# IuvenisSapiens/Qwen3-TTS-Rust

Measured on AMD Instinct MI355X. Metric: audio-seconds generated per second (aggregate over GPUs) = concurrent real-time streams; RTF and first-chunk latency from the single-utterance leg, higher is better.
Workload: dtype i8

## Files before the change

qwen3-tts-rust_amd/csrc/codec.hip:

```cpp
#include "codec.h"
#include "../../include/q3tts.h"
#include "gguf.h"
#include <cmath>
#include <cstdlib>
#include <map>

namespace q3 {

typedef float f32x16 __attribute__((ext_vector_type(16)));

enum { EPI_NONE = 0, EPI_GELU = 1, EPI_RES_SCALE = 2, EPI_RES = 3, EPI_SNAKE = 4 };

struct GemmArgs {
    const float* A; int lda;
    int cin, dil;
    const float* W;
    const float* wscale;
    const float* bias;
    float* out; int ldo;
    int M, N, K;
    int epi; const float* res; int ldr; const float* scale;
    const float *snake_ea, *snake_ib;
    float* ws;
    int a_segT, a_skip; int o_segT; long long o_skip; int r_segT; long long r_skip;
// ... 124 lines not shown
            const int e = tid + i * 256, r = e % BN, qd = e / BN;
            if (e < BN * 4) { Bs[4 * qd + 0][r] = rb[i].x; Bs[4 * qd + 1][r] = rb[i].y; Bs[4 * qd + 2][r] = rb[i].z; Bs[4 * qd + 3][r] = rb[i].w; }
        }
    };
    fetch(kbeg);
    for (int k0 = kbeg; k0 < kend; k0 += BK) {
        stash();
        __syncthreads();
        if (k0 + BK < kend) fetch(k0 + BK);
#pragma unroll
        for (int kk = 0; kk < BK; kk += 2) {
            const float a = As[kk + (lane >> 5)][wm * 32 + (lane & 31)];
            const float b = Bs[kk + (lane >> 5)][wn * 32 + (lane & 31)];
            acc = __builtin_amdgcn_mfma_f32_32x32x2f32(a, b, acc, 0, 0, 0);
        }
        __syncthreads();
    }
    const int col = n0 + wn * 32 + (lane & 31);
    if (col < g.N) {
#pragma unroll
        for (int r = 0; r < 16; r++) {
            const int row = m0 + wm * 32 + (r & 3) + 8 * (r >> 2) + 4 * (lane >> 5);
            if (row < g.M) {
                if (ksplit > 1) g.ws[((size_t)blockIdx.z * g.M + row) * g.N + col] = acc[r];
                else gemm_store(g, row, col, gemm_epilogue(g, acc[r], row, col));
            }
        }
    }
}
typedef _Float16 h8v __attribute__((ext_vector_type(8)));
typedef _Float16 h4v __attribute__((ext_vector_type(4)));
template <int MR, int EPL, bool SPLIT>
__global__ void __launch_bounds__(256) k_conv_gemm_h(GemmArgs g, const _Float16* __restrict__ Wh, const _Float16* __restrict__ Wl) {
    constexpr int BM = 64 * MR, BN = 64, BK = 32, LD = 40;
    constexpr int NA = BM * 8 / 256;
    constexpr int CLD = BN + 4;
    struct Stage { _Float16 Ah[BM][LD], Al[BM][LD], Bh[BN][LD], Bl[BN][LD]; };
    union Shared { Stage s; float Ct[EPL ? BM : 1][CLD]; };
    __shared__ __attribute__((aligned(16))) Shared sh;
    auto& Ah = sh.s.Ah; auto& Al = sh.s.Al; auto& Bh = sh.s.Bh; auto& Bl = sh.s.Bl;
    const int tid = threadIdx.x, lane = tid & 63, wave = tid >> 6;
    const int wm = wave >> 1, wn = wave & 1;
    const int m0 = blockIdx.y * BM, n0 = blockIdx.x * BN;
    const int ksplit = gridDim.z, kper = g.K / ksplit, kbeg = blockIdx.z * kper, kend = kbeg + kper;
    f32x16 acc[MR];
#pragma unroll
    for (int t = 0; t < MR; t++)
#pragma unroll
        for (int i = 0; i < 16; i++) acc[t][i] = 0.0f;
    float4 ra[NA];
    uint4 rh, rl;
    int arow[NA];
#pragma unroll
    for (int i = 0; i < NA; i++) { int mm = m0 + (tid + i * 256) / 8; mm = mm < g.M ? mm : g.M - 1; arow[i] = mm + seg_of(mm, g.a_segT) * g.a_skip; }
    const int wrow = (n0 + tid / 4 < g.N) ? n0 + tid / 4 : g.N - 1, wk = 8 * (tid & 3);
    const int scol = n0 + wn * 32 + (lane & 31);
    const float wsc = g.wscale[scol < g.N ? scol : g.N - 1];
    auto fetch = [&](int k0) {
        const int j = k0 / g.cin, ci0 = k0 % g.cin;
#pragma unroll
        for (int i = 0; i < NA; i++) {
            const int kq = (tid + i * 256) % 8;
            const size_t row = (size_t)(arow[i] + j * g.dil);
            if constexpr (SPLIT) ra[i] = load_a4_split_raw(g, row, ci0 + 4 * kq);
            else ra[i] = *reinterpret_cast<const float4*>(g.A + row * g.lda + ci0 + 4 * kq);
        }
        rh = *reinterpret_cast<const uint4*>(Wh + (size_t)wrow * g.K + k0 + wk);
        rl = *reinterpret_cast<const uint4*>(Wl + (size_t)wrow * g.K + k0 + wk);
    };
    auto stash = [&]() {
#pragma unroll
        for (int i = 0; i < NA; i++) {
            const int e = tid + i * 256, r = e / 8, kq = e % 8;
            if constexpr (SPLIT) {
                *reinterpret_cast<float2*>(&Ah[r][4 * kq]) = make_float2(ra[i].x, ra[i].y);
                *reinterpret_cast<float2*>(&Al[r][4 * kq]) = make_float2(ra[i].z, ra[i].w);
            } else {
                const float x[4] = {ra[i].x, ra[i].y, ra[i].z, ra[i].w};
                h4v hi, lo;
#pragma unroll
                for (int c = 0; c < 4; c++) { hi[c] = (_Float16)x[c]; lo[c] = (_Float16)(x[c] - (float)hi[c]); }
                *reinterpret_cast<h4v*>(&Ah[r][4 * kq]) = hi;
                *reinterpret_cast<h4v*>(&Al[r][4 * kq]) = lo;
            }
        }
        *reinterpret_cast<uint4*>(&Bh[tid / 4][wk]) = rh;
        *reinterpret_cast<uint4*>(&Bl[tid / 4][wk]) = rl;
    };
    auto multiply = [&]() {
#pragma unroll
        for (int kk = 0; kk < BK; kk += 16) {
            const int ko = kk + 8 * (lane >> 5);
            const h8v bh = *reinterpret_cast<const h8v*>(&Bh[wn * 32 + (lane & 31)][ko]);
            const h8v bl = *reinterpret_cast<const h8v*>(&Bl[wn * 32 + (lane & 31)][ko]);
#pragma unroll
            for (int t = 0; t < MR; t++) {
                const int ar = (wm * MR + t) * 32 + (lane & 31);
                const h8v ah = *reinterpret_cast<const h8v*>(&Ah[ar][ko]);
                const h8v al = *reinterpret_cast<const h8v*>(&Al[ar][ko]);
                acc[t] = __builtin_amdgcn_mfma_f32_32x32x16_f16(al, bh, acc[t], 0, 0, 0);
                acc[t] = __builtin_amdgcn_mfma_f32_32x32x16_f16(ah, bl, acc[t], 0, 0, 0);
                acc[t] = __builtin_amdgcn_mfma_f32_32x32x16_f16(ah, bh, acc[t], 0, 0, 0);
            }
        }
    };
    auto lds_barrier = [] { asm volatile("s_waitcnt lgkmcnt(0)\n\ts_barrier" ::: "memory"); };
    fetch(kbeg);
    int k0 = kbeg;
    for (; k0 + BK < kend; k0 += BK) {
        stash();
        lds_barrier();
        fetch(k0 + BK);
        multiply();
        lds_barrier();
    }
    stash();
    lds_barrier();
    multiply();
#pragma unroll
    for (int t = 0; t < MR; t++)
#pragma unroll
        for (int r = 0; r < 16; r++) acc[t][r] *= wsc;
    __syncthreads();
    if constexpr (EPL != 0) {
        auto& Ct = sh.Ct;
#pragma unroll
        for (int t = 0; t < MR; t++)
#pragma unroll
            for (int r = 0; r < 16; r++) Ct[(wm * MR + t) * 32 + (r & 3) + 8 * (r >> 2) + 4 * (lane >> 5)][wn * 32 + (lane & 31)] = acc[t][r];
        __syncthreads();
        for (int e = tid; e < BM * (BN / 4); e += 256) {
            const int rl = e / (BN / 4), cl = (e % (BN / 4)) * 4, row = m0 + rl, col = n0 + cl;
            if (row >= g.M || col >= g.N) continue;
            const float4 t4 = *reinterpret_cast<const float4*>(&Ct[rl][cl]);
            if (ksplit > 1) *reinterpret_cast<float4*>(g.ws + ((size_t)blockIdx.z * g.M + row) * g.N + col) = t4;
            else gemm_epilogue_store4(g, t4, row, col);
        }
    } else {
        const int col = n0 + wn * 32 + (lane & 31);
        if (col < g.N) {
#pragma unroll
            for (int t = 0; t < MR; t++)
#pragma unroll
                for (int r = 0; r < 16; r++) {
                    const int row = m0 + (wm * MR + t) * 32 + (r & 3) + 8 * (r >> 2) + 4 * (lane >> 5);
                    if (row < g.M) {
                        if (ksplit > 1) g.ws[((size_t)blockIdx.z * g.M + row) * g.N + col] = acc[t][r];
                        else gemm_store(g, row, col, gemm_epilogue(g, acc[t][r], row, col));
                    }
                }
        }
    }
}
template <int MR, int NT, int BK, int EPL, int PF, bool SPLIT>
__global__ void __launch_bounds__(256) k_conv_gemm_h3(GemmArgs g, const _Float16* __restrict__ Wh, const _Float16* __restrict__ Wl) {
    constexpr int BM = 128 * MR, BN = 32 * NT, LD = BK + 8;
    constexpr int KQ = BK / 4, KC = BK / 8;
    constexpr int NA = BM * KQ / 256;
    constexpr int NB = (BN * KC + 255) / 256;
    constexpr int CLD = BN + 4;
    struct Stage { _Float16 Ah[BM][LD], Al[BM][LD], Bh[BN][LD], Bl[BN][LD]; };
    union Shared { Stage s; float Ct[EPL ? BM : 1][CLD]; };
    __shared__ __attribute__((aligned(16))) Shared sh;
    auto& Ah = sh.s.Ah; auto& Al = sh.s.Al; auto& Bh = sh.s.Bh; auto& Bl = sh.s.Bl;
    const int tid = threadIdx.x, lane = tid & 63, wave = tid >> 6;
    int tile_m = blockIdx.y, tile_n = blockIdx.x;
    if (g.xcd_swizzle) {
        const int nwg = gridDim.x * gridDim.y, orig = blockIdx.y * gridDim.x + blockIdx.x;
        const int xcd = orig & 7, q8 = nwg >> 3, r8 = nwg & 7;
        const int wgid = (xcd < r8 ? xcd * (q8 + 1) : r8 * (q8 + 1) + (xcd - r8) * q8) + (orig >> 3);
        tile_n = wgid % gridDim.x; tile_m = wgid / gridDim.x;
    }
    const int m0 = tile_m * BM, n0 = tile_n * BN;
    const int ksplit = gridDim.z, kper = g.K / ksplit, kbeg = blockIdx.z * kper, kend = kbeg + kper;
    f32x16 acc[MR][NT];
#pragma unroll
    for (int t = 0; t < MR; t++)
#pragma unroll
        for (int u = 0; u < NT; u++)
#pragma unroll
            for (int i = 0; i < 16; i++) acc[t][u][i] = 0.0f;
    int arow[NA];
#pragma unroll
    for (int i = 0; i < NA; i++) { int mm = m0 + (tid + i * 256) / KQ; mm = mm < g.M ? mm : g.M - 1; arow[i] = mm + seg_of(mm, g.a_segT) * g.a_skip; }
    struct Regs { float4 ra[NA]; uint4 rh[NB], rl[NB]; };
    auto fetch = [&](Regs& s, int k0) {
        const int j = k0 / g.cin, ci0 = k0 % g.cin;
#pragma unroll
        for (int i = 0; i < NA; i++) {
            const int kq = (tid + i * 256) % KQ;
            const size_t row = (size_t)(arow[i] + j * g.dil);
            if constexpr (SPLIT) s.ra[i] = load_a4_split_raw(g, row, ci0 + 4 * kq);
            else s.ra[i] = *reinterpret_cast<const float4*>(g.A + row * g.lda + ci0 + 4 * kq);
        }
#pragma unroll
        for (int i = 0; i < NB; i++) {
            int e = tid + i * 256;
            e = e < BN * KC ? e : e - 256;
            const int r = e / KC, wk = 8 * (e % KC);
            s.rh[i] = *reinterpret_cast<const uint4*>(Wh + (size_t)(n0 + r) * g.K + k0 + wk);
            s.rl[i] = *reinterpret_cast<const uint4*>(Wl + (size_t)(n0 + r) * g.K + k0 + wk);
        }
    };
    auto stash = [&](const Regs& s) {
#pragma unroll
        for (int i = 0; i < NA; i++) {
            const int e = tid + i * 256, r = e / KQ, kq = e % KQ;
            if constexpr (SPLIT) {
                *reinterpret_cast<float2*>(&Ah[r][4 * kq]) = make_float2(s.ra[i].x, s.ra[i].y);
                *reinterpret_cast<float2*>(&Al[r][4 * kq]) = make_float2(s.ra[i].z, s.ra[i].w);
            } else {
                const float x[4] = {s.ra[i].x, s.ra[i].y, s.ra[i].z, s.ra[i].w};
                h4v hi, lo;
#pragma unroll
                for (int c = 0; c < 4; c++) { hi[c] = (_Float16)x[c]; lo[c] = (_Float16)(x[c] - (float)hi[c]); }
                *reinterpret_cast<h4v*>(&Ah[r][4 * kq]) = hi;
                *reinterpret_cast<h4v*>(&Al[r][4 * kq]) = lo;
            }
        }
#pragma unroll
        for (int i = 0; i < NB; i++) {
            const int e = tid + i * 256, r = e / KC, wk = 8 * (e % KC);
            if (e < BN * KC) { *reinterpret_cast<uint4*>(&Bh[r][wk]) = s.rh[i]; *reinterpret_cast<uint4*>(&Bl[r][wk]) = s.rl[i]; }
        }
    };
    auto multiply = [&]() {
#pragma unroll
        for (int kk = 0; kk < BK; kk += 16) {
            const int ko = kk + 8 * (lane >> 5);
            if constexpr (MR == 1) {
                const int ar = wave * 32 + (lane & 31);
                const h8v ah = *reinterpret_cast<const h8v*>(&Ah[ar][ko]);
                const h8v al = *reinterpret_cast<const h8v*>(&Al[ar][ko]);
#pragma unroll
                for (int u = 0; u < NT; u++) {
                    const h8v bh = *reinterpret_cast<const h8v*>(&Bh[u * 32 + (lane & 31)][ko]);
                    const h8v bl = *reinterpret_cast<const h8v*>(&Bl[u * 32 + (lane & 31)][ko]);
                    acc[0][u] = __builtin_amdgcn_mfma_f32_32x32x16_f16(al, bh, acc[0][u], 0, 0, 0);
                    acc[0][u] = __builtin_amdgcn_mfma_f32_32x32x16_f16(ah, bl, acc[0][u], 0, 0, 0);
                    acc[0][u] = __builtin_amdgcn_mfma_f32_32x32x16_f16(ah, bh, acc[0][u], 0, 0, 0);
                }
            } else {
                h8v bh[NT], bl[NT];
#pragma unroll
                for (int u = 0; u < NT; u++) {
                    bh[u] = *reinterpret_cast<const h8v*>(&Bh[u * 32 + (lane & 31)][ko]);
                    bl[u] = *reinterpret_cast<const h8v*>(&Bl[u * 32 + (lane & 31)][ko]);
                }
#pragma unroll
                for (int t = 0; t < MR; t++) {
                    const int ar = (wave * MR + t) * 32 + (lane & 31);
                    const h8v ah = *reinterpret_cast<const h8v*>(&Ah[ar][ko]);
                    const h8v al = *reinterpret_cast<const h8v*>(&Al[ar][ko]);
#pragma unroll
                    for (int u = 0; u < NT; u++) {
                        acc[t][u] = __builtin_amdgcn_mfma_f32_32x32x16_f16(al, bh[u], acc[t][u], 0, 0, 0);
                        acc[t][u] = __builtin_amdgcn_mfma_f32_32x32x16_f16(ah, bl[u], acc[t][u], 0, 0, 0);
                        acc[t][u] = __builtin_amdgcn_mfma_f32_32x32x16_f16(ah, bh[u], acc[t][u], 0, 0, 0);
                    }
                    __builtin_amdgcn_sched_barrier(0);
                }
            }
        }
    };
    auto lds_barrier = [] { asm volatile("s_waitcnt lgkmcnt(0)\n\ts_barrier" ::: "memory"); };
    float wsc[NT];
#pragma unroll
    for (int u = 0; u < NT; u++) wsc[u] = g.wscale[n0 + u * 32 + (lane & 31)];
    Regs st[PF];
#pragma unroll
    for (int j = 0; j < PF; j++)
        if (kbeg + j * BK < kend) fetch(st[j], kbeg + j * BK);
    int k0 = kbeg;
    for (; k0 + 2 * PF * BK <= kend; k0 += PF * BK) {
#pragma unroll
        for (int j = 0; j < PF; j++) {
            stash(st[j]);
            lds_barrier();
            fetch(st[j], k0 + (j + PF) * BK);
            multiply();
            lds_barrier();
        }
    }
    for (; k0 < kend; k0 += PF * BK) {
#pragma unroll
        for (int j = 0; j < PF; j++) {
            if (k0 + j * BK < kend) {
                stash(st[j]);
                lds_barrier();
                if (k0 + (j + PF) * BK < kend) fetch(st[j], k0 + (j + PF) * BK);
                multiply();
                lds_barrier();
            }
        }
    }
#pragma unroll
    for (int u = 0; u < NT; u++)
#pragma unroll
        for (int t = 0; t < MR; t++)
#pragma unroll
            for (int r = 0; r < 16; r++) acc[t][u][r] *= wsc[u];
    __syncthreads();
    auto epilogue_rows = [&](const f32x16 (&a)[NT], int row0) {
#pragma unroll
        for (int r = 0; r < 16; r++) {
            const int row = row0 + (r & 3) + 8 * (r >> 2) + 4 * (lane >> 5);
            if (row < g.M) {
#pragma unroll
                for (int u = 0; u < NT; u++) {
                    const int col = n0 + u * 32 + (lane & 31);
                    if (col < g.N) {
                        if (ksplit > 1) g.ws[((size_t)blockIdx.z * g.M + row) * g.N + col] = a[u][r];
                        else gemm_store(g, row, col, gemm_epilogue(g, a[u][r], row, col));
                    }
                }
            }
        }
    };
    if constexpr (EPL != 0 && MR == 1) {
        auto& Ct = sh.Ct;
#pragma unroll
        for (int u = 0; u < NT; u++)
#pragma unroll
            for (int r = 0; r < 16; r++) Ct[wave * 32 + (r & 3) + 8 * (r >> 2) + 4 * (lane >> 5)][u * 32 + (lane & 31)] = acc[0][u][r];
        __syncthreads();
        constexpr int C4 = BN / 4;
        for (int e = tid; e < BM * C4; e += 256) {
            const int rl = e / C4, col = n0 + (e % C4) * 4, row = m0 + rl;
            if (row >= g.M) continue;
            const float4 t4 = *reinterpret_cast<const float4*>(&Ct[rl][(e % C4) * 4]);
            if (ksplit > 1) *reinterpret_cast<float4*>(g.ws + ((size_t)blockIdx.z * g.M + row) * g.N + col) = t4;
            else gemm_epilogue_store4(g, t4, row, col);
        }
    } else {
        epilogue_rows(acc[0], m0 + wave * MR * 32);
        if constexpr (MR > 1) epilogue_rows(acc[1], m0 + (wave * MR + 1) * 32);
    }
    static_assert(MR <= 2, "one epilogue call per row tile");
}
__global__ void __launch_bounds__(256) k_splitk_reduce4(GemmArgs g, int ksplit) {
    const size_t i = ((size_t)blockIdx.x * 256 + threadIdx.x) * 4, mn = (size_t)g.M * g.N;
    if (i >= mn) return;
    const int row = (int)(i / g.N), col = (int)(i % g.N);
    float4 v = *reinterpret_cast<const float4*>(g.ws + i);
    for (int s = 1; s < ksplit; s++) {
        const float4 w = *reinterpret_cast<const float4*>(g.ws + (size_t)s * mn + i);
        v.x += w.x; v.y += w.y; v.z += w.z; v.w += w.w;
    }
    gemm_epilogue_store4(g, v, row, col);
}
__global__ void __launch_bounds__(256) k_splitk_reduce(GemmArgs g, int ksplit) {
    const size_t i = (size_t)blockIdx.x * 256 + threadIdx.x;
    if (i >= (size_t)g.M * g.N) return;
    const int row = (int)(i / g.N), col = (int)(i % g.N);
    float v = g.ws[i];
    for (int s = 1; s < ksplit; s++) v += g.ws[(size_t)s * g.M * g.N + i];
    gemm_store(g, row, col, gemm_epilogue(g, v, row, col));
}

template <int MT>
__global__ void __launch_bounds__(512) k_skinny_gemm(GemmArgs g) {
    constexpr int KT = 512;
    __shared__ __attribute__((aligned(16))) float As[MT][KT];
    const int tid = threadIdx.x, lane = tid & 63, wave = tid >> 6;
    const int n = blockIdx.x * 8 + wave;
    const int nn = n < g.N ? n : g.N - 1;
    float acc[MT];
#pragma unroll
    for (int m = 0; m < MT; m++) acc[m] = 0.0f;
    for (int k0 = 0; k0 < g.K; k0 += KT) {
        const int kt = (g.K - k0) < KT ? (g.K - k0) : KT;
        float4 w4[2];
#pragma unroll
        for (int i = 0; i < 2; i++) {
            const int kk = 4 * (lane + 64 * i);
            w4[i] = (kk < kt) ? *reinterpret_cast<const float4*>(g.W + (size_t)nn * g.K + k0 + kk) : make_float4(0.f, 0.f, 0.f, 0.f);
        }
        __syncthreads();
        for (int e = tid; e < MT * (KT / 4); e += 512) {
            const int m = e / (KT / 4), kk = 4 * (e % (KT / 4));
            float4 v = make_float4(0.f, 0.f, 0.f, 0.f);
            if (m < g.M && kk < kt) {
                const int kg = k0 + kk, j = kg / g.cin, ci = kg % g.cin;
                v = load_a4(g, (size_t)(m + seg_of(m, g.a_segT) * g.a_skip + j * g.dil), ci);
            }
            *reinterpret_cast<float4*>(&As[m][kk]) = v;
        }
        __syncthreads();
#pragma unroll
        for (int i = 0; i < 2; i++) {
            const int kk = 4 * (lane + 64 * i);
#pragma unroll
            for (int m = 0; m < MT; m++) {
                const float4 a = *reinterpret_cast<const float4*>(&As[m][kk]);
                acc[m] += w4[i].x * a.x + w4[i].y * a.y + w4[i].z * a.z + w4[i].w * a.w;
            }
        }
    }
    float mine = 0.0f;
#pragma unroll
    for (int m = 0; m < MT; m++) {
        float v = acc[m];
        for (int o = 32; o >= 1; o >>= 1) v += __shfl_xor(v, o);
        if (lane == m) mine = v;
    }
    if (lane < MT && lane < g.M && n < g.N) gemm_store(g, lane, n, gemm_epilogue(g, mine, lane, n));
}
static const bool g_codec_f32 = [] { const char* e = std::getenv("Q3_CODEC_F32"); return e && e[0] == '1'; }();
struct GemmPlan { int form, ks, red; };
static GemmPlan plan_gemm(const GemmArgs& g, size_t ws_floats, bool has_split_w) {
    if (g.M <= 16) return GemmPlan{g.M <= 4 ? Q3TTS_GEMM_SKINNY4 : g.M <= 8 ? Q3TTS_GEMM_SKINNY8 : Q3TTS_GEMM_SKINNY16, 1, -1};
    const bool small = g.M <= 32;
    const int tiles = small ? ((g.N + 127) / 128) * ((g.M + 31) / 32) : ((g.N + 63) / 64) * ((g.M + 63) / 64);
    int ksplit = 1;
    while (tiles * ksplit < 256 && ksplit < 16 && (g.K / (ksplit * 2)) % 16 == 0 && g.K / (ksplit * 2) >= 128 &&
           (size_t)(ksplit * 2) * g.M * g.N <= ws_floats) ksplit *= 2;
    const bool ws_a16 = (reinterpret_cast<uintptr_t>(g.ws) & 15) == 0;
    static const int h3_min_wgs = [] { const char* e = std::getenv("Q3_CODEC_H3_MIN_WGS"); return e ? atoi(e) : 128; }();
    static const int h3_max_n = [] { const char* e = std::getenv("Q3_CODEC_H3_MAXN"); return e ? atoi(e) : 1 << 30; }();
    static const int epl_on = [] { const char* e = std::getenv("Q3_CODEC_H3_EPL"); return e ? atoi(e) : 1; }();
    static const int h3_wgs = [] { const char* e = std::getenv("Q3_CODEC_H3_WGS"); return e ? atoi(e) : 0; }();
    static const int h3_min_tiles = [] { const char* e = std::getenv("Q3_CODEC_H3_MIN_TILES"); return e ? atoi(e) : 96; }();
    if (!small && has_split_w && !g_codec_f32 && g.cin % 32 == 0 && h3_min_wgs > 0 && g.N % 96 == 0 && g.N <= h3_max_n) {
        const int tiles3 = (g.N / 96) * ((g.M + 127) / 128);
        const bool vec_ok = epl_on && epilogue4_ok(g) && ws_a16;
        int ks = 1;
        if (vec_ok && h3_wgs > 0 && tiles3 >= h3_min_tiles && tiles3 < h3_wgs) {
            static const int cand[] = {2, 3, 4, 6, 7, 8, 12, 14, 16};
            for (int c : cand) {
                if (g.K % c != 0 || (g.K / c) % 32 != 0 || g.K / c < 256 || (size_t)c * g.M * g.N > ws_floats) continue;
                ks = c;
                if (tiles3 * c >= h3_wgs) break;
            }
        }
        if (tiles3 * ks >= h3_min_wgs) return GemmPlan{vec_ok ? Q3TTS_GEMM_H3_EPL : Q3TTS_GEMM_H3, ks, ks > 1 ? 1 : -1};
    }
    if (!small && has_split_w && !g_codec_f32 && g.cin % 32 == 0) {
        static const int big_m = [] { const char* e = std::getenv("Q3_CODEC_BM128"); return e ? atoi(e) : 1024; }();
        const bool tall = g.M >= big_m && g.N >= 512 && ((g.N + 63) / 64) * ((g.M + 127) / 128) >= 160;
        const int t2 = tall ? ((g.N + 63) / 64) * ((g.M + 127) / 128) : tiles;
        static const int wg_target = [] { const char* e = std::getenv("Q3_CODEC_WGS"); return e ? atoi(e) : 256; }();
        int ks = 1;
        while (t2 * ks < wg_target && ks < 16 && (g.K / (ks * 2)) % 32 == 0 && g.K / (ks * 2) >= 128 && (size_t)(ks * 2) * g.M * g.N <= ws_floats) ks *= 2;
        static const int epl4 = [] { const char* e = std::getenv("Q3_CODEC_EPL4"); return e ? atoi(e) : 1; }();
        const bool vec_ok = epl4 && epilogue4_ok(g) && ws_a16;
        const int form = tall ? (vec_ok ? Q3TTS_GEMM_H2_EPL : Q3TTS_GEMM_H2) : (vec_ok ? Q3TTS_GEMM_H1_EPL : Q3TTS_GEMM_H1);
        return GemmPlan{form, ks, ks > 1 ? (vec_ok ? 1 : 0) : -1};
    }
    return GemmPlan{small ? Q3TTS_GEMM_F32_1 : Q3TTS_GEMM_F32_2, ksplit, ksplit > 1 ? 0 : -1};
}
static const char* gemm_plan_error(const GemmArgs& g, const GemmPlan& p, size_t ws_floats, bool has_split_w) {
    const int f = p.form;
    if (f < Q3TTS_GEMM_SKINNY4 || f > Q3TTS_GEMM_H3_EPL) return "unknown GEMM form";
    if (g.M < 1 || g.N < 1 || g.cin < 4 || g.K % g.cin != 0 || g.dil < 1) return "bad GEMM shape";
    if (g.cin % 4 != 0 || g.lda % 4 != 0 || g.lda < g.cin) return "A rows need cin % 4 == 0 and lda % 4 == 0, lda >= cin";
    if (p.ks < 1 || g.K % p.ks != 0) return "ksplit must divide K";
    const bool skinny = f <= Q3TTS_GEMM_SKINNY16, f32 = f == Q3TTS_GEMM_F32_1 || f == Q3TTS_GEMM_F32_2, h3 = f >= Q3TTS_GEMM_H3;
    const bool epl = f == Q3TTS_GEMM_H1_EPL || f == Q3TTS_GEMM_H2_EPL || f == Q3TTS_GEMM_H3_EPL;
    const bool ws_a16 = (reinterpret_cast<uintptr_t>(g.ws) & 15) == 0;
    if (skinny) {
        if (g.M > (f == Q3TTS_GEMM_SKINNY4 ? 4 : f == Q3TTS_GEMM_SKINNY8 ? 8 : 16)) return "skinny form: M exceeds its row count";
        if (p.ks != 1) return "skinny form: no split-K";
        return nullptr;
    }
    if (f32 && (g.cin % 16 != 0 || (g.K / p.ks) % 16 != 0)) return "f32 form: cin and K / ksplit must be multiples of 16";
    if (!f32) {
        if (!has_split_w || !g.wscale) return "split-f16 form without split weights";
        if (g.cin % 32 != 0 || (g.K / p.ks) % 32 != 0) return "split-f16 form: cin and K / ksplit must be multiples of 32";
        if (h3 && g.N % 96 != 0) return "h3 form: N must be a multiple of 96";
        if (epl && !(epilogue4_ok(g) && ws_a16)) return "16-byte epilogue form: pointers / strides not 16-byte aligned or N % 4 != 0";
    }
    if (p.ks > 1) {
        if (p.ks > 64) return "ksplit too large";
        if ((size_t)p.ks * g.M * g.N > ws_floats) return "split-K workspace too small";
        if (p.red != 0 && p.red != 1) return "split-K needs a reducer (0 or 1)";
        if (p.red == 1 && !(epilogue4_ok(g) && ws_a16)) return "k_splitk_reduce4: pointers / strides not 16-byte aligned or N % 4 != 0";
    } else if (p.red != -1) return "a reducer without split-K";
    return nullptr;
}
static void launch_gemm(hipStream_t st, const GemmArgs& g, const GemmPlan& p, const _Float16* wh, const _Float16* wl) {
    const dim3 b256(256);
    const unsigned ks = (unsigned)p.ks;
#define Q3_H(MRV, EPLV, GRID) do { if (g.a_split) hipLaunchKernelGGL((k_conv_gemm_h<MRV, EPLV, true>), GRID, b256, 0, st, g, wh, wl); \
                                   else hipLaunchKernelGGL((k_conv_gemm_h<MRV, EPLV, false>), GRID, b256, 0, st, g, wh, wl); } while (0)
#define Q3_H3(EPLV, PFV) do { if (g.a_split) hipLaunchKernelGGL((k_conv_gemm_h3<1, 3, 32, EPLV, PFV, true>), grid3, b256, 0, st, g, wh, wl); \
                              else hipLaunchKernelGGL((k_conv_gemm_h3<1, 3, 32, EPLV, PFV, false>), grid3, b256, 0, st, g, wh, wl); } while (0)
    const dim3 grid_sk((g.N + 7) / 8), grid_t((g.N + 63) / 64, (g.M + 127) / 128, ks), grid_s((g.N + 63) / 64, (g.M + 63) / 64, ks);
    const dim3 grid3(g.N / 96, (g.M + 127) / 128, ks);
    switch (p.form) {
    case Q3TTS_GEMM_SKINNY4: hipLaunchKernelGGL((k_skinny_gemm<4>), grid_sk, dim3(512), 0, st, g); break;
    case Q3TTS_GEMM_SKINNY8: hipLaunchKernelGGL((k_skinny_gemm<8>), grid_sk, dim3(512), 0, st, g); break;
    case Q3TTS_GEMM_SKINNY16: hipLaunchKernelGGL((k_skinny_gemm<16>), grid_sk, dim3(512), 0, st, g); break;
    case Q3TTS_GEMM_F32_1: hipLaunchKernelGGL((k_conv_gemm<1>), dim3((g.N + 127) / 128, (g.M + 31) / 32, ks), b256, 0, st, g); break;
    case Q3TTS_GEMM_F32_2: hipLaunchKernelGGL((k_conv_gemm<2>), dim3((g.N + 63) / 64, (g.M + 63) / 64, ks), b256, 0, st, g); break;
    case Q3TTS_GEMM_H1: Q3_H(1, 0, grid_s); break;
    case Q3TTS_GEMM_H1_EPL: Q3_H(1, 1, grid_s); break;
    case Q3TTS_GEMM_H2: Q3_H(2, 0, grid_t); break;
    case Q3TTS_GEMM_H2_EPL: Q3_H(2, 1, grid_t); break;
    case Q3TTS_GEMM_H3: Q3_H3(0, 1); break;
    case Q3TTS_GEMM_H3_EPL: Q3_H3(1, 1); break;
    default: throw Error("unknown GEMM form");
    }
#undef Q3_H
#undef Q3_H3
    if (p.ks > 1) {
        const size_t n = (size_t)g.M * g.N;
        if (p.red == 1) hipLaunchKernelGGL(k_splitk_reduce4, dim3((unsigned)((n / 4 + 255) / 256)), b256, 0, st, g, p.ks);
        else hipLaunchKernelGGL(k_splitk_reduce, dim3((unsigned)((n + 255) / 256)), b256, 0, st, g, p.ks);
    }
}
static int xcd_swizzle_on() { static const int on = [] { const char* e = std::getenv("Q3_CODEC_XCD"); return e ? atoi(e) : 1; }(); return on; }
static void gemm(hipStream_t st, GemmArgs g, float* ws, size_t ws_floats, const _Float16* wh = nullptr, const _Float16* wl = nullptr) {
    g.ws = ws;
    g.xcd_swizzle = xcd_swizzle_on();
    launch_gemm(st, g, plan_gemm(g, ws_floats, wh != nullptr), wh, wl);
}

struct RowMap { int segT, skip, off; };
__device__ __forceinline__ size_t map_row(const RowMap& m, int r) { return (size_t)r + (size_t)(m.segT == SEG_NONE ? 0 : r / m.segT) * m.skip + m.off; }
static RowMap plain_map() { return RowMap{SEG_NONE, 0, 0}; }

__global__ void k_rvq_sum(const int64_t* __restrict__ codes, const float* const* __restrict__ cb, int n_q, int cb_size, int cb_dim,
                          float* __restrict__ out, int ldo, RowMap om) {
    const int t = blockIdx.y, d = blockIdx.x * 256 + threadIdx.x;
    if (d >= cb_dim) return;
    float acc = 0.0f;
    for (int q = 0; q < n_q; q++) {
        long long c = codes[(size_t)t * n_q + q];
        c = c < 0 ? 0 : (c >= cb_size ? cb_size - 1 : c);
        acc += cb[q][(size_t)c * cb_dim + d];
    }
    out[map_row(om, t) * ldo + d] = acc;
}
__global__ void __launch_bounds__(256) k_rmsnorm_rows(const float* __restrict__ x, int ldx, const float* __restrict__ g, int C, float eps,
                                                      float* __restrict__ y, int ldy) {
    __shared__ float red[4];
    const int t = blockIdx.x;
    float s = 0.0f;
    for (int c = threadIdx.x; c < C; c += 256) { const float v = x[(size_t)t * ldx + c]; s += v * v; }
    for (int o = 32; o >= 1; o >>= 1) s += __shfl_xor(s, o);
    if ((threadIdx.x & 63) == 0) red[threadIdx.x >> 6] = s;
    __syncthreads();
    const float tot = red[0] + red[1] + red[2] + red[3];
    const float sc = 1.0f / sqrtf(tot / (float)C + eps);
    for (int c = threadIdx.x; c < C; c += 256) y[(size_t)t * ldy + c] = x[(size_t)t * ldx + c] * sc * g[c];
}
__global__ void __launch_bounds__(256) k_layernorm_rows(const float* __restrict__ x, int ldx, const float* __restrict__ w,
                                                        const float* __restrict__ b, int C, float eps, float* __restrict__ y, int ldy) {
    __shared__ float red[8];
    const int t = blockIdx.x;
    float s = 0.0f;
    for (int c = threadIdx.x; c < C; c += 256) s += x[(size_t)t * ldx + c];
    for (int o = 32; o >= 1; o >>= 1) s += __shfl_xor(s, o);
    if ((threadIdx.x & 63) == 0) red[threadIdx.x >> 6] = s;
    __syncthreads();
    const float mu = (red[0] + red[1] + red[2] + red[3]) / (float)C;
    float v = 0.0f;
    for (int c = threadIdx.x; c < C; c += 256) { const float dlt = x[(size_t)t * ldx + c] - mu; v += dlt * dlt; }
    for (int o = 32; o >= 1; o >>= 1) v += __shfl_xor(v, o);
    if ((threadIdx.x & 63) == 0) red[4 + (threadIdx.x >> 6)] = v;
    __syncthreads();
    const float var = (red[4] + red[5] + red[6] + red[7]) / (float)C;
    const float inv = 1.0f / sqrtf(var + eps);
    for (int c = threadIdx.x; c < C; c += 256) y[(size_t)t * ldy + c] = (x[(size_t)t * ldx + c] - mu) * inv * w[c] + b[c];
}
__global__ void k_codec_rope_append(float* __restrict__ qkv, int ld, int H, int hd, const float* __restrict__ cs, const float* __restrict__ sn,
                                    const int64_t* __restrict__ meta, int G, int T0, float* __restrict__ kext, float* __restrict__ vext, RowMap om) {
    const int r = blockIdx.y, e = blockIdx.x * 256 + threadIdx.x, half = hd / 2;
    if (e >= H / 2) return;
    const int head = e / half, i = e % half;
    const long long p = meta[2 * G + r / T0] + (r % T0);
    const float c = cs[(size_t)p * half + i], s = sn[(size_t)p * half + i];
    const size_t o = map_row(om, r) * H;
    float* row = qkv + (size_t)r * ld;
    {
        float* v = row + head * hd;
        const float a = v[i], b = v[i + half];
        v[i] = a * c - b * s; v[i + half] = b * c + a * s;
    }
    {
        float* v = row + H + head * hd;
        const float a = v[i], b = v[i + half];
        const float x = a * c - b * s, y = b * c + a * s;
        v[i] = x; v[i + half] = y;
        kext[o + head * hd + i] = x; kext[o + head * hd + i + half] = y;
    }
    vext[o + e] = row[2 * H + e];
    vext[o + e + H / 2] = row[2 * H + e + H / 2];
}
__global__ void __launch_bounds__(64) k_codec_attn(const float* __restrict__ qkv, int ld, int H, int hd, const float* __restrict__ kext,
                                                   const float* __restrict__ vext, const int64_t* __restrict__ meta, int G, int T0, int W,
                                                   float* __restrict__ out, int ldo) {
    __shared__ float p_s[128];
    __shared__ float q_s[128];
    const int head = blockIdx.x, r = blockIdx.y, lane = threadIdx.x;
    const int g = r / T0, t = r % T0;
    const int kvl = (int)meta[G + g];
    const size_t seg = (size_t)g * (W - 1 + T0);
    const int j1 = W - 1 + t, jv = W - 1 - kvl, j0 = t > jv ? t : jv, nk = j1 - j0 + 1;
    for (int d = lane; d < hd; d += 64) q_s[d] = qkv[(size_t)r * ld + head * hd + d];
    __syncthreads();
    const float scale = 1.0f / sqrtf((float)hd);
    float mx = -INFINITY;
    for (int jj = lane; jj < nk; jj += 64) {
        const float* kr = kext + (seg + j0 + jj) * H + head * hd;
        float a = 0.0f;
        if ((hd & 3) == 0) {
            for (int d = 0; d < hd; d += 4) {
                const float4 kk = *reinterpret_cast<const float4*>(kr + d);
                a += q_s[d] * kk.x; a += q_s[d + 1] * kk.y; a += q_s[d + 2] * kk.z; a += q_s[d + 3] * kk.w;
            }
        } else for (int d = 0; d < hd; d++) a += q_s[d] * kr[d];
        a *= scale;
        p_s[jj] = a;
        mx = fmaxf(mx, a);
    }
    for (int o = 32; o >= 1; o >>= 1) mx = fmaxf(mx, __shfl_xor(mx, o));
    float den = 0.0f;
    for (int jj = lane; jj < nk; jj += 64) { const float e = expf(p_s[jj] - mx); p_s[jj] = e; den += e; }
    for (int o = 32; o >= 1; o >>= 1) den += __shfl_xor(den, o);
    __syncthreads();
    for (int d = lane; d < hd; d += 64) {
        float a = 0.0f;
        for (int jj = 0; jj < nk; jj++) a += p_s[jj] * vext[(seg + j0 + jj) * H + head * hd + d];
        out[(size_t)r * ldo + head * hd + d] = a / den;
    }
}
__global__ void k_swiglu_rows(const float* __restrict__ gu, int ff, float* __restrict__ out) {
    const int t = blockIdx.y, c = blockIdx.x * 256 + threadIdx.x;
    if (c >= ff) return;
    const float g = gu[(size_t)t * 2 * ff + c], u = gu[(size_t)t * 2 * ff + ff + c];
    out[(size_t)t * ff + c] = (g / (1.0f + expf(-g))) * u;
}
__global__ void k_dwconv7(const float* __restrict__ in_ext, int C, const float* __restrict__ w, const float* __restrict__ b,
                          float* __restrict__ out, RowMap im) {
    const int t = blockIdx.y, c = blockIdx.x * 256 + threadIdx.x;
    if (c >= C) return;
    const size_t r0 = map_row(im, t);
    float a = b[c];
#pragma unroll
    for (int j = 0; j < 7; j++) a += w[c * 7 + j] * in_ext[(r0 + j) * C + c];
    out[(size_t)t * C + c] = a;
}
__global__ void k_snake(const float* __restrict__ src, float* __restrict__ dst, int C, const float* __restrict__ ea,
                        const float* __restrict__ inv_eb, size_t n4, RowMap dm, int split) {
    const size_t i = (size_t)blockIdx.x * 256 + threadIdx.x;
    if (i >= n4) return;
    const int c4 = C >> 2, c = (int)(i % c4) * 4, r = (int)(i / c4);
    const float4 v = reinterpret_cast<const float4*>(src)[i];
    const float4 a = *reinterpret_cast<const float4*>(ea + c), b = *reinterpret_cast<const float4*>(inv_eb + c);
    const float s0 = snake_sin(v.x * a.x), s1 = snake_sin(v.y * a.y), s2 = snake_sin(v.z * a.z), s3 = snake_sin(v.w * a.w);
    const float4 y = make_float4(v.x + b.x * (s0 * s0), v.y + b.y * (s1 * s1), v.z + b.z * (s2 * s2), v.w + b.w * (s3 * s3));
    float* drow = dst + map_row(dm, r) * C;
// ... 780 lines not shown
```

Before: 695.3.

## Pipeline h3 codec GEMM weights via direct global-to-LDS loads in a 3-stage ring

Rewrites the h3 split-f16 conv GEMM so weight tiles are copied straight from global memory into LDS with global_load_lds across a 3-stage ring buffer, with hand-placed vmcnt waits. Activation tiles move to per-wave LDS slices with an XOR swizzle and are prefetched two tiles ahead through inline-asm async loads. The output staging for the 16-byte epilogue is split into two halves so it fits inside the smaller operand footprint. The aim is to overlap weight and activation traffic with MFMA work and cut register staging and bank conflicts, at the cost of fragile hand-counted waitcnt logic and the loss of the generic MR/PF template parameters.

```diff
diff --git a/qwen3-tts-rust_amd/csrc/codec.hip b/qwen3-tts-rust_amd/csrc/codec.hip
--- a/qwen3-tts-rust_amd/csrc/codec.hip
+++ b/qwen3-tts-rust_amd/csrc/codec.hip
@@ -300,17 +300,27 @@
         }
     }
 }
-template <int MR, int NT, int BK, int EPL, int PF, bool SPLIT>
+constexpr int H3_STAGES = 3;
+typedef float f32x4 __attribute__((ext_vector_type(4)));
+typedef float f32x2 __attribute__((ext_vector_type(2)));
+__device__ __forceinline__ f32x4 gload16_async(const void* p) { f32x4 v; asm volatile("global_load_dwordx4 %0, %1, off" : "=v"(v) : "v"(p) : "memory"); return v; }
+__device__ __forceinline__ f32x2 gload8_async(const void* p) { f32x2 v; asm volatile("global_load_dwordx2 %0, %1, off" : "=v"(v) : "v"(p) : "memory"); return v; }
+template <int N> __device__ __forceinline__ void vm_wait() { asm volatile("s_waitcnt vmcnt(%0)" :: "n"(N) : "memory"); }
+template <int N> __device__ __forceinline__ void vm_wait_regs(f32x4 (&r)[4]) {
+    asm volatile("s_waitcnt vmcnt(%4)" : "+v"(r[0]), "+v"(r[1]), "+v"(r[2]), "+v"(r[3]) : "n"(N) : "memory");
+}
+template <int EPL, int ST, bool SPLIT>
 __global__ void __launch_bounds__(256) k_conv_gemm_h3(GemmArgs g, const _Float16* __restrict__ Wh, const _Float16* __restrict__ Wl) {
-    constexpr int BM = 128 * MR, BN = 32 * NT, LD = BK + 8;
-    constexpr int KQ = BK / 4, KC = BK / 8;
-    constexpr int NA = BM * KQ / 256;
-    constexpr int NB = (BN * KC + 255) / 256;
-    constexpr int CLD = BN + 4;
-    struct Stage { _Float16 Ah[BM][LD], Al[BM][LD], Bh[BN][LD], Bl[BN][LD]; };
-    union Shared { Stage s; float Ct[EPL ? BM : 1][CLD]; };
-    __shared__ __attribute__((aligned(16))) Shared sh;
-    auto& Ah = sh.s.Ah; auto& Al = sh.s.Al; auto& Bh = sh.s.Bh; auto& Bl = sh.s.Bl;
+    constexpr int BM = 128, NT = 3, BN = 32 * NT, BK = 32;
+    constexpr int BPLANE = BN * BK * 2, BSTAGE = 2 * BPLANE;
+    constexpr int APLANE = 32 * BK * 2, ASLICE = 2 * APLANE;
+    constexpr int NBL = BSTAGE / 1024 / 4;
+    constexpr int NAL = SPLIT ? 8 : 4;
+    constexpr int CLD = BN + 4, CROWS = 64;
+    constexpr int OPS = ST * BSTAGE + 4 * ASLICE;
+    static_assert(BSTAGE % 4096 == 0 && ST >= 2, "whole DMA blocks per wave; a ring needs 2 stages");
+    static_assert(!EPL || CROWS * CLD * 4 <= OPS, "the staged output half fits in the operand footprint");
+    __shared__ __attribute__((aligned(16))) unsigned char smem[OPS];
     const int tid = threadIdx.x, lane = tid & 63, wave = tid >> 6;
     int tile_m = blockIdx.y, tile_n = blockIdx.x;
     if (g.xcd_swizzle) {
@@ -320,136 +330,129 @@
         tile_n = wgid % gridDim.x; tile_m = wgid / gridDim.x;
     }
     const int m0 = tile_m * BM, n0 = tile_n * BN;
-    const int ksplit = gridDim.z, kper = g.K / ksplit, kbeg = blockIdx.z * kper, kend = kbeg + kper;
-    f32x16 acc[MR][NT];
-#pragma unroll
-    for (int t = 0; t < MR; t++)
-#pragma unroll
-        for (int u = 0; u < NT; u++)
-#pragma unroll
-            for (int i = 0; i < 16; i++) acc[t][u][i] = 0.0f;
-    int arow[NA];
-#pragma unroll
-    for (int i = 0; i < NA; i++) { int mm = m0 + (tid + i * 256) / KQ; mm = mm < g.M ? mm : g.M - 1; arow[i] = mm + seg_of(mm, g.a_segT) * g.a_skip; }
-    struct Regs { float4 ra[NA]; uint4 rh[NB], rl[NB]; };
-    auto fetch = [&](Regs& s, int k0) {
-        const int j = k0 / g.cin, ci0 = k0 % g.cin;
-#pragma unroll
-        for (int i = 0; i < NA; i++) {
-            const int kq = (tid + i * 256) % KQ;
+    const int ksplit = gridDim.z, kper = g.K / ksplit, kbeg = blockIdx.z * kper, nt = kper / BK;
+    f32x16 acc[NT];
+#pragma unroll
+    for (int u = 0; u < NT; u++)
+#pragma unroll
+        for (int i = 0; i < 16; i++) acc[u][i] = 0.0f;
+    int arow[4];
+#pragma unroll
+    for (int i = 0; i < 4; i++) { int mm = m0 + wave * 32 + (lane >> 3) + 8 * i; mm = mm < g.M ? mm : g.M - 1; arow[i] = mm + seg_of(mm, g.a_segT) * g.a_skip; }
+    unsigned char* const aslice = smem + ST * BSTAGE + wave * ASLICE;
+    auto swz = [](int r, int c) { return r * 64 + ((c ^ ((r >> 2) & 3)) << 4); };
+    auto tile_k = [&](int t) { return kbeg + (t < nt ? t : nt - 1) * BK; };
+    auto issue_w = [&](int t) {
+        const int k0 = tile_k(t);
+        unsigned char* const stage = smem + (t % ST) * BSTAGE;
+#pragma unroll
+        for (int i = 0; i < NBL; i++) {
+            const int q = i * 4 + wave, pl = q >= BN / 16 ? 1 : 0, r = 16 * (q - pl * (BN / 16)) + (lane >> 2);
+            const int c = (lane & 3) ^ ((lane >> 4) & 3);
+            const _Float16* src = (pl ? Wl : Wh) + (size_t)(n0 + r) * g.K + k0 + 8 * c;
+            __builtin_amdgcn_global_load_lds((__attribute__((address_space(1))) void*)src, (__attribute__((address_space(3))) void*)(stage + q * 1024), 16, 0, 0);
+        }
+    };
+    auto fetch_a = [&](f32x4 (&ra)[4], int t) {
+        const int k0 = tile_k(t), j = k0 / g.cin, ci = k0 % g.cin + 4 * (lane & 7);
+#pragma unroll
+        for (int i = 0; i < 4; i++) {
             const size_t row = (size_t)(arow[i] + j * g.dil);
-            if constexpr (SPLIT) s.ra[i] = load_a4_split_raw(g, row, ci0 + 4 * kq);
-            else s.ra[i] = *reinterpret_cast<const float4*>(g.A + row * g.lda + ci0 + 4 * kq);
-        }
-#pragma unroll
-        for (int i = 0; i < NB; i++) {
-            int e = tid + i * 256;
-            e = e < BN * KC ? e : e - 256;
-            const int r = e / KC, wk = 8 * (e % KC);
-            s.rh[i] = *reinterpret_cast<const uint4*>(Wh + (size_t)(n0 + r) * g.K + k0 + wk);
-            s.rl[i] = *reinterpret_cast<const uint4*>(Wl + (size_t)(n0 + r) * g.K + k0 + wk);
+            if constexpr (SPLIT) {
+                const _Float16* base = reinterpret_cast<const _Float16*>(g.A + row * g.lda);
+                const f32x2 hi = gload8_async(base + ci), lo = gload8_async(base + g.cin + ci);
+                ra[i] = f32x4{hi.x, hi.y, lo.x, lo.y};
+            } else ra[i] = gload16_async(g.A + row * g.lda + ci);
         }
     };
-    auto stash = [&](const Regs& s) {
-#pragma unroll
-        for (int i = 0; i < NA; i++) {
-            const int e = tid + i * 256, r = e / KQ, kq = e % KQ;
+    auto stash_a = [&](const f32x4 (&ra)[4]) {
+#pragma unroll
+        for (int i = 0; i < 4; i++) {
+            const int r = (lane >> 3) + 8 * i, kq = lane & 7, o = swz(r, kq >> 1) + 8 * (kq & 1);
             if constexpr (SPLIT) {
-                *reinterpret_cast<float2*>(&Ah[r][4 * kq]) = make_float2(s.ra[i].x, s.ra[i].y);
-                *reinterpret_cast<float2*>(&Al[r][4 * kq]) = make_float2(s.ra[i].z, s.ra[i].w);
+                *reinterpret_cast<float2*>(aslice + o) = make_float2(ra[i].x, ra[i].y);
+                *reinterpret_cast<float2*>(aslice + APLANE + o) = make_float2(ra[i].z, ra[i].w);
             } else {
-                const float x[4] = {s.ra[i].x, s.ra[i].y, s.ra[i].z, s.ra[i].w};
+                const float x[4] = {ra[i].x, ra[i].y, ra[i].z, ra[i].w};
                 h4v hi, lo;
 #pragma unroll
                 for (int c = 0; c < 4; c++) { hi[c] = (_Float16)x[c]; lo[c] = (_Float16)(x[c] - (float)hi[c]); }
-                *reinterpret_cast<h4v*>(&Ah[r][4 * kq]) = hi;
-                *reinterpret_cast<h4v*>(&Al[r][4 * kq]) = lo;
+                *reinterpret_cast<h4v*>(aslice + o) = hi;
+                *reinterpret_cast<h4v*>(aslice + APLANE + o) = lo;
             }
         }
-#pragma unroll
-        for (int i = 0; i < NB; i++) {
-            const int e = tid + i * 256, r = e / KC, wk = 8 * (e % KC);
-            if (e < BN * KC) { *reinterpret_cast<uint4*>(&Bh[r][wk]) = s.rh[i]; *reinterpret_cast<uint4*>(&Bl[r][wk]) = s.rl[i]; }
-        }
     };
-    auto multiply = [&]() {
+    auto multiply = [&](int t) {
+        const unsigned char* const stage = smem + (t % ST) * BSTAGE;
 #pragma unroll
         for (int kk = 0; kk < BK; kk += 16) {
-            const int ko = kk + 8 * (lane >> 5);
-            if constexpr (MR == 1) {
-                const int ar = wave * 32 + (lane & 31);
-                const h8v ah = *reinterpret_cast<const h8v*>(&Ah[ar][ko]);
-                const h8v al = *reinterpret_cast<const h8v*>(&Al[ar][ko]);
-#pragma unroll
-                for (int u = 0; u < NT; u++) {
-                    const h8v bh = *reinterpret_cast<const h8v*>(&Bh[u * 32 + (lane & 31)][ko]);
-                    const h8v bl = *reinterpret_cast<const h8v*>(&Bl[u * 32 + (lane & 31)][ko]);
-                    acc[0][u] = __builtin_amdgcn_mfma_f32_32x32x16_f16(al, bh, acc[0][u], 0, 0, 0);
-                    acc[0][u] = __builtin_amdgcn_mfma_f32_32x32x16_f16(ah, bl, acc[0][u], 0, 0, 0);
-                    acc[0][u] = __builtin_amdgcn_mfma_f32_32x32x16_f16(ah, bh, acc[0][u], 0, 0, 0);
-                }
-            } else {
-                h8v bh[NT], bl[NT];
-#pragma unroll
-                for (int u = 0; u < NT; u++) {
-                    bh[u] = *reinterpret_cast<const h8v*>(&Bh[u * 32 + (lane & 31)][ko]);
-                    bl[u] = *reinterpret_cast<const h8v*>(&Bl[u * 32 + (lane & 31)][ko]);
-                }
-#pragma unroll
-                for (int t = 0; t < MR; t++) {
-                    const int ar = (wave * MR + t) * 32 + (lane & 31);
-                    const h8v ah = *reinterpret_cast<const h8v*>(&Ah[ar][ko]);
-                    const h8v al = *reinterpret_cast<const h8v*>(&Al[ar][ko]);
-#pragma unroll
-                    for (int u = 0; u < NT; u++) {
-                        acc[t][u] = __builtin_amdgcn_mfma_f32_32x32x16_f16(al, bh[u], acc[t][u], 0, 0, 0);
-                        acc[t][u] = __builtin_amdgcn_mfma_f32_32x32x16_f16(ah, bl[u], acc[t][u], 0, 0, 0);
-                        acc[t][u] = __builtin_amdgcn_mfma_f32_32x32x16_f16(ah, bh[u], acc[t][u], 0, 0, 0);
-                    }
-                    __builtin_amdgcn_sched_barrier(0);
-                }
+            const int o = swz(lane & 31, kk / 8 + (lane >> 5));
+            const h8v ah = *reinterpret_cast<const h8v*>(aslice + o);
+            const h8v al = *reinterpret_cast<const h8v*>(aslice + APLANE + o);
+#pragma unroll
+            for (int u = 0; u < NT; u++) {
+                const h8v bh = *reinterpret_cast<const h8v*>(stage + u * 32 * 64 + o);
+                const h8v bl = *reinterpret_cast<const h8v*>(stage + BPLANE + u * 32 * 64 + o);
+                acc[u] = __builtin_amdgcn_mfma_f32_32x32x16_f16(al, bh, acc[u], 0, 0, 0);
+                acc[u] = __builtin_amdgcn_mfma_f32_32x32x16_f16(ah, bl, acc[u], 0, 0, 0);
+                acc[u] = __builtin_amdgcn_mfma_f32_32x32x16_f16(ah, bh, acc[u], 0, 0, 0);
             }
         }
     };
     auto lds_barrier = [] { asm volatile("s_waitcnt lgkmcnt(0)\n\ts_barrier" ::: "memory"); };
+    constexpr int VM_W = NAL + (ST - 2) * (NBL + NAL), VM_A = NBL;
+    static_assert(VM_W < 64, "vmcnt is 6 bits");
     float wsc[NT];
 #pragma unroll
     for (int u = 0; u < NT; u++) wsc[u] = g.wscale[n0 + u * 32 + (lane & 31)];
-    Regs st[PF];
-#pragma unroll
-    for (int j = 0; j < PF; j++)
-        if (kbeg + j * BK < kend) fetch(st[j], kbeg + j * BK);
-    int k0 = kbeg;
-    for (; k0 + 2 * PF * BK <= kend; k0 += PF * BK) {
-#pragma unroll
-        for (int j = 0; j < PF; j++) {
-            stash(st[j]);
-            lds_barrier();
-            fetch(st[j], k0 + (j + PF) * BK);
-            multiply();
-            lds_barrier();
-        }
-    }
-    for (; k0 < kend; k0 += PF * BK) {
-#pragma unroll
-        for (int j = 0; j < PF; j++) {
-            if (k0 + j * BK < kend) {
-                stash(st[j]);
-                lds_barrier();
-                if (k0 + (j + PF) * BK < kend) fetch(st[j], k0 + (j + PF) * BK);
-                multiply();
-                lds_barrier();
+    f32x4 ra[4];
+    for (int t = 0; t < ST - 1; t++) issue_w(t);
+    fetch_a(ra, 0);
+    vm_wait_regs<0>(ra);
+    stash_a(ra);
+    fetch_a(ra, 1);
+    vm_wait_regs<0>(ra);
+    for (int t = 0; t < nt; t++) {
+        vm_wait<VM_W>();
+        lds_barrier();
+        issue_w(t + ST - 1);
+        __builtin_amdgcn_sched_barrier(0);
+        multiply(t);
+        __builtin_amdgcn_sched_barrier(0);
+        vm_wait_regs<VM_A>(ra);
+        stash_a(ra);
+        fetch_a(ra, t + 2);
+        __builtin_amdgcn_sched_barrier(0);
+    }
+    vm_wait_regs<0>(ra);
+    __syncthreads();
+#pragma unroll
+    for (int u = 0; u < NT; u++)
+#pragma unroll
+        for (int r = 0; r < 16; r++) acc[u][r] *= wsc[u];
+    if constexpr (EPL != 0) {
+        float (*Ct)[CLD] = reinterpret_cast<float (*)[CLD]>(smem);
+        constexpr int C4 = BN / 4;
+#pragma unroll
+        for (int h = 0; h < 2; h++) {
+            if ((wave >> 1) == h) {
+#pragma unroll
+                for (int u = 0; u < NT; u++)
+#pragma unroll
+                    for (int r = 0; r < 16; r++) Ct[(wave & 1) * 32 + (r & 3) + 8 * (r >> 2) + 4 * (lane >> 5)][u * 32 + (lane & 31)] = acc[u][r];
             }
-        }
-    }
-#pragma unroll
-    for (int u = 0; u < NT; u++)
-#pragma unroll
-        for (int t = 0; t < MR; t++)
-#pragma unroll
-            for (int r = 0; r < 16; r++) acc[t][u][r] *= wsc[u];
-    __syncthreads();
-    auto epilogue_rows = [&](const f32x16 (&a)[NT], int row0) {
+            __syncthreads();
+            for (int e = tid; e < CROWS * C4; e += 256) {
+                const int rl = e / C4, col = n0 + (e % C4) * 4, row = m0 + h * CROWS + rl;
+                if (row >= g.M) continue;
+                const float4 t4 = *reinterpret_cast<const float4*>(&Ct[rl][(e % C4) * 4]);
+                if (ksplit > 1) *reinterpret_cast<float4*>(g.ws + ((size_t)blockIdx.z * g.M + row) * g.N + col) = t4;
+                else gemm_epilogue_store4(g, t4, row, col);
+            }
+            if (h == 0) __syncthreads();
+        }
+    } else {
+        const int row0 = m0 + wave * 32;
 #pragma unroll
         for (int r = 0; r < 16; r++) {
             const int row = row0 + (r & 3) + 8 * (r >> 2) + 4 * (lane >> 5);
@@ -457,34 +460,12 @@
 #pragma unroll
                 for (int u = 0; u < NT; u++) {
                     const int col = n0 + u * 32 + (lane & 31);
-                    if (col < g.N) {
-                        if (ksplit > 1) g.ws[((size_t)blockIdx.z * g.M + row) * g.N + col] = a[u][r];
-                        else gemm_store(g, row, col, gemm_epilogue(g, a[u][r], row, col));
-                    }
+                    if (ksplit > 1) g.ws[((size_t)blockIdx.z * g.M + row) * g.N + col] = acc[u][r];
+                    else gemm_store(g, row, col, gemm_epilogue(g, acc[u][r], row, col));
                 }
             }
         }
-    };
-    if constexpr (EPL != 0 && MR == 1) {
-        auto& Ct = sh.Ct;
-#pragma unroll
-        for (int u = 0; u < NT; u++)
-#pragma unroll
-            for (int r = 0; r < 16; r++) Ct[wave * 32 + (r & 3) + 8 * (r >> 2) + 4 * (lane >> 5)][u * 32 + (lane & 31)] = acc[0][u][r];
-        __syncthreads();
-        constexpr int C4 = BN / 4;
-        for (int e = tid; e < BM * C4; e += 256) {
-            const int rl = e / C4, col = n0 + (e % C4) * 4, row = m0 + rl;
-            if (row >= g.M) continue;
-            const float4 t4 = *reinterpret_cast<const float4*>(&Ct[rl][(e % C4) * 4]);
-            if (ksplit > 1) *reinterpret_cast<float4*>(g.ws + ((size_t)blockIdx.z * g.M + row) * g.N + col) = t4;
-            else gemm_epilogue_store4(g, t4, row, col);
-        }
-    } else {
-        epilogue_rows(acc[0], m0 + wave * MR * 32);
-        if constexpr (MR > 1) epilogue_rows(acc[1], m0 + (wave * MR + 1) * 32);
-    }
-    static_assert(MR <= 2, "one epilogue call per row tile");
+    }
 }
 __global__ void __launch_bounds__(256) k_splitk_reduce4(GemmArgs g, int ksplit) {
     const size_t i = ((size_t)blockIdx.x * 256 + threadIdx.x) * 4, mn = (size_t)g.M * g.N;
@@ -631,8 +612,8 @@
     const unsigned ks = (unsigned)p.ks;
 #define Q3_H(MRV, EPLV, GRID) do { if (g.a_split) hipLaunchKernelGGL((k_conv_gemm_h<MRV, EPLV, true>), GRID, b256, 0, st, g, wh, wl); \
                                    else hipLaunchKernelGGL((k_conv_gemm_h<MRV, EPLV, false>), GRID, b256, 0, st, g, wh, wl); } while (0)
-#define Q3_H3(EPLV, PFV) do { if (g.a_split) hipLaunchKernelGGL((k_conv_gemm_h3<1, 3, 32, EPLV, PFV, true>), grid3, b256, 0, st, g, wh, wl); \
-                              else hipLaunchKernelGGL((k_conv_gemm_h3<1, 3, 32, EPLV, PFV, false>), grid3, b256, 0, st, g, wh, wl); } while (0)
+#define Q3_H3(EPLV) do { if (g.a_split) hipLaunchKernelGGL((k_conv_gemm_h3<EPLV, H3_STAGES, true>), grid3, b256, 0, st, g, wh, wl); \
+                         else hipLaunchKernelGGL((k_conv_gemm_h3<EPLV, H3_STAGES, false>), grid3, b256, 0, st, g, wh, wl); } while (0)
     const dim3 grid_sk((g.N + 7) / 8), grid_t((g.N + 63) / 64, (g.M + 127) / 128, ks), grid_s((g.N + 63) / 64, (g.M + 63) / 64, ks);
     const dim3 grid3(g.N / 96, (g.M + 127) / 128, ks);
     switch (p.form) {
@@ -645,8 +626,8 @@
     case Q3TTS_GEMM_H1_EPL: Q3_H(1, 1, grid_s); break;
     case Q3TTS_GEMM_H2: Q3_H(2, 0, grid_t); break;
     case Q3TTS_GEMM_H2_EPL: Q3_H(2, 1, grid_t); break;
-    case Q3TTS_GEMM_H3: Q3_H3(0, 1); break;
-    case Q3TTS_GEMM_H3_EPL: Q3_H3(1, 1); break;
+    case Q3TTS_GEMM_H3: Q3_H3(0); break;
+    case Q3TTS_GEMM_H3_EPL: Q3_H3(1); break;
     default: throw Error("unknown GEMM form");
     }
 #undef Q3_H
```

Result: no change. 700.9 (median of 6 runs) (+0.8%).
